# huj31415/nbody3d-webgpu

Hardware: AMD Instinct MI355X
Metric: pair-interactions/s (higher is better)
Workload: dtype f32; 1 GPU; N=262144 Plummer sphere, dt=1e-3, G=1, eps2=1e-4, i-sharded over 1 GPU(s); n=262144, kernel_variant=f32pk_symw_ipl16_j1_w2048_r32t128, parallelism=1gpu

## Files before the change

include/nbody3d_hip.h:

```cpp
#ifndef NBODY3D_HIP_H
#define NBODY3D_HIP_H

#include <stddef.h>
#include <stdint.h>

#ifdef __cplusplus
extern "C" {
#endif
#if defined(__GNUC__)
#pragma GCC visibility push(default)
#endif

#define NB_ABI_VERSION 2u
#define NB_ABI_MINOR 4u

typedef struct nb_sim nb_sim;

typedef enum nb_status {
    NB_OK = 0,
    NB_ERR_INVALID = 1,
    NB_ERR_NO_DEVICE = 2,
    NB_ERR_HIP = 3,
    NB_ERR_STATE = 4,
    NB_ERR_NOMEM = 5,
    NB_ERR_COMM = 6,
    NB_NOT_READY = 7
} nb_status;

typedef enum nb_precision { NB_F32 = 0, NB_F64 = 1 } nb_precision;

#define NB_FLAG_EXT_STREAM 1u
#define NB_FLAG_LDS_ONLY 4u
#define NB_FLAG_NO_FUSE 8u
#define NB_FLAG_POISON 16u

#define NB_FLAG_JPK_FENCED 32u

#define NB_FLAG_NO_SYM 64u

#define NB_FLAG_SYM_SHARD 128u

#define NB_FLAG_WHOLE_SWEEPS 256u

#define NB_FLAG_SINGLE_SWEEPS 512u

typedef enum nb_array { NB_BODIES = 0, NB_VEL = 1, NB_ACCEL = 2, NB_JERK = 3  } nb_array;

typedef enum nb_integrator { NB_INT_LEAPFROG = 0, NB_INT_HERMITE4 = 1 } nb_integrator;

typedef struct nb_config {
    uint32_t struct_size;
    uint32_t n;
    uint32_t precision;
    uint32_t tile;
    double eps2;
    int32_t device;
    uint32_t shard_begin;
    uint32_t shard_count;
    void *ext_stream;
    void *ext_bodies;
    uint32_t force_variant;
    uint32_t jsplit;
    uint32_t flags;
    uint32_t layer_budget_mib;
    uint32_t integrator;
    uint32_t reserved[3];
} nb_config;
// ... 55 lines not shown

int nb_enable_timing(nb_sim *s, int on);
int nb_kernel_times(nb_sim *s, double *force_ms, double *integrate_ms,
                    uint32_t *launches);
int nb_step_times(nb_sim *s, double *force_ms, double *integrate_ms, double *exchange_ms,
                  uint32_t *launches);
typedef struct nb_step_timing {
    uint32_t struct_size;
    uint32_t launches;
    double force_ms;
    double sym_reduce_ms;
    double reduce_scatter_ms;
    double integrate_ms;
    double allgather_ms;
    double span_ms;
    uint32_t reduce_scatters;
    uint32_t allgathers;
} nb_step_timing;
int nb_step_times2(nb_sim *s, nb_step_timing *out);
int nb_integrate_pass(nb_sim *s, uint32_t reps, double *avg_ms);
int nb_force_pass(nb_sim *s, uint32_t reps, double *avg_ms);

const char *nb_variant_name(nb_sim *s);

int nb_shape_info(nb_sim *s, uint32_t *jsplit, uint32_t *j_per_split, uint32_t *own_split0,
                  uint32_t *own_splits);



int nb_download_jerk(nb_sim *s, void *jerk);

int nb_upload_derivs(nb_sim *s, const void *accel, const void *jerk);

#define NB_BLOCK_FROZEN 1u
typedef struct nb_block_steps {
    uint32_t struct_size;
    uint32_t max_level;
    uint32_t min_level;
    uint32_t flags;
    double   eta;
} nb_block_steps;
int nb_set_block_steps(nb_sim *s, const nb_block_steps *cfg );

struct nb_block_stats {
    uint32_t struct_size, enabled;
    uint64_t outer_steps, block_steps, body_steps;
// ... 55 lines not shown
```

nbody3d-webgpu_amd/csrc/kernels/symmetric.hip.h:

```cpp
#pragma once

namespace nb {

template <typename T> struct SymRowT { T x, y, z; };
using SymRow = SymRowT<float>;

constexpr uint32_t kFlushSteps = 4096;

template <int NG>
__device__ __forceinline__ void flush_resident_sums(float (*hi)[64], const int lane, const bool flushed, nb_f2 (&ax)[NG], nb_f2 (&ay)[NG], nb_f2 (&az)[NG])
{
    if (flushed) {
#pragma unroll
        for (int c = 0; c < NG; ++c) {
            hi[6 * c + 0][lane] += ax[c].x; hi[6 * c + 1][lane] += ay[c].x; hi[6 * c + 2][lane] += az[c].x;
            hi[6 * c + 3][lane] += ax[c].y; hi[6 * c + 4][lane] += ay[c].y; hi[6 * c + 5][lane] += az[c].y;
        }
    } else {
#pragma unroll
        for (int c = 0; c < NG; ++c) {
            hi[6 * c + 0][lane] = ax[c].x; hi[6 * c + 1][lane] = ay[c].x; hi[6 * c + 2][lane] = az[c].x;
            hi[6 * c + 3][lane] = ax[c].y; hi[6 * c + 4][lane] = ay[c].y; hi[6 * c + 5][lane] = az[c].y;
        }
    }
#pragma unroll
    for (int c = 0; c < NG; ++c) { ax[c] = nb_f2{0, 0}; ay[c] = nb_f2{0, 0}; az[c] = nb_f2{0, 0}; }
}

__device__ __forceinline__ float wave_rot1(float v)
{
// ... 151 lines not shown
template <int TAIL>
__device__ __forceinline__ void symw_record_and_tail(const uint32_t* rec_at, nb_u4& rec, uint32_t (&tail)[TAIL])
{
    static_assert(TAIL == 1 || TAIL == 4, "f32: eps2; f64: G, eps2");
    constexpr int kTailOffset = 4 * 8 + 6 * 4;
    if constexpr (TAIL == 1) {
        asm volatile("s_load_dwordx4 %0, %2, 0x0\n\ts_load_dword %1, %3, %4\n\ts_waitcnt lgkmcnt(0)"
                     : "=&s"(rec), "=&s"(tail[0]) : "s"(rec_at), "s"(__builtin_amdgcn_kernarg_segment_ptr()), "n"(kTailOffset) : "memory");
    } else {
        nb_u4 t;
        asm volatile("s_load_dwordx4 %0, %2, 0x0\n\ts_load_dwordx4 %1, %3, %4\n\ts_waitcnt lgkmcnt(0)"
                     : "=&s"(rec), "=&s"(t) : "s"(rec_at), "s"(__builtin_amdgcn_kernarg_segment_ptr()), "n"(kTailOffset) : "memory");
        tail[0] = t.x; tail[1] = t.y; tail[2] = t.z; tail[3] = t.w;
    }
}

__device__ __forceinline__ SymWK symw_plan_words(uint32_t S, uint32_t cps, uint32_t W, uint32_t ups, uint32_t nsb, uint32_t zc, uint32_t r_layer0, uint32_t t_layer0)
{
    const uint32_t H = (nsb - 1u) >> 1, n_hi = (nsb & 1u) ? 0u : nsb >> 1;
    const uint32_t total_lo = (H + 1u) * cps + zc, total_hi = total_lo + (n_hi ? cps : 0u);
    return SymWK{(nsb + (zc ? 1u : 0u)) * S, nsb, W, total_hi, total_lo, n_hi, zc, ups, r_layer0, t_layer0};
}

template <int NG, int J, bool PAIR>
__device__ __forceinline__ void symw_sweeps(const uint32_t* __restrict__ gtab, const float4* __restrict__ bodies, SymRow* __restrict__ partial, SymRow* __restrict__ spill,
                                            SYMW_PLAN_PARAMS, uint32_t* __restrict__ queue, const uint32_t npieces, const uint32_t pieces_off)
{
    static_assert(!PAIR || J == 1, "paired sweeps: one traveler per lane and sweep");
    constexpr uint32_t S = 128u * NG;
    constexpr int GW = NG < 4 ? NG : 4;
    constexpr uint32_t CH = 64u * J;
    constexpr uint32_t CPS = S / CH;
    const SymWK pl = symw_plan_words(S, CPS, W_, ups_, nsb_, zc_, r_layer0_, t_layer0_);
    const int lane = threadIdx.x & 63, wi = threadIdx.x >> 6;
    const uint32_t w = __builtin_amdgcn_readfirstlane(blockIdx.x * 4u + wi);
    const bool active = w < pl.W;
    NB_STAMP(0);
    __shared__ float red[4][6 * NG][64];
    __shared__ uint32_t fin[4];
    const uint32_t ups = pl.ups, ush = (uint32_t)__builtin_ctz(ups), ustep = 64u >> ush,
                   tab1 = 2u * (pl.np / S);
    nb_u4 rec;
    uint32_t tail[1];
    symw_record_and_tail(gtab + tab1 + 4u * (active ? w : 0u), rec, tail);
    const float eps2 = __builtin_bit_cast(float, tail[0]);
    const nb_f2 e2 = nb_f2{eps2, eps2};
    const uint32_t first_lo = pl.n_hi * pl.total_hi, first_z = first_lo + (pl.nsb - pl.n_hi) * pl.total_lo;
    const uint32_t slot = rec.w;
    NB_STAMP_LIGHT(1);
    bool first_part = true;

    auto run = [&](uint32_t u, const uint32_t uend, const uint32_t piece_layer) -> uint32_t {
        uint32_t gfin = ~0u;
        while (u < uend) {
            const uint32_t p = u >> ush;
            uint32_t g, k, total;
            if (p < first_lo) { g = p / pl.total_hi; k = p - g * pl.total_hi; total = pl.total_hi; }
            else if (p < first_z) { const uint32_t r = p - first_lo; g = pl.n_hi + r / pl.total_lo; k = r - (g - pl.n_hi) * pl.total_lo; total = pl.total_lo; }
            else { g = pl.nsb; k = p - first_z; total = pl.zc; }
            const uint32_t ring = g < pl.nsb ? total - CPS - pl.zc : 0u;
            const uint32_t both_end = g < pl.nsb ? ring + pl.zc : 0u;
            uint32_t ug_end = (p - k + total) * ups;
// ... 25 lines not shown
                    since = 0;
                }
                since += pair ? 128u : s1 - s0;
                const bool sym = k < both_end, zsweep = k >= ring && sym;
                const uint32_t d = k / CPS;
                uint32_t tb = g + 1 + d;
                if (tb >= pl.nsb) tb -= pl.nsb;
                const uint32_t tstart = k < ring ? tb * S + (k % CPS) * CH : zsweep ? pl.nsb * S + (k - ring) * CH : g * S + (k - both_end) * CH;
                const uint32_t zrow = g * pl.zc + (k - ring);
                ++k;
                if constexpr (PAIR) {
                    if (pair) {
                        const bool zsweep1 = k >= ring;
                        const uint32_t d1 = k / CPS;
                        uint32_t tb1 = g + 1 + d1;
                        if (tb1 >= pl.nsb) tb1 -= pl.nsb;
                        const uint32_t tstart1 = zsweep1 ? pl.nsb * S + (k - ring) * CH : tb1 * S + (k % CPS) * CH;
                        const uint32_t zrow1 = g * pl.zc + (k - ring);
                        ++k;
                        const float4 t0 = ld4(bodies + tstart + lane), t1 = ld4(bodies + tstart1 + lane);
                        nb_f2 tx = nb_f2{t0.x, t1.x}, ty = nb_f2{t0.y, t1.y}, tz = nb_f2{t0.z, t1.z}, tm = nb_f2{t0.w, t1.w};
                        float bx0 = 0, bx1 = 0, by0 = 0, by1 = 0, bz0 = 0, bz1 = 0;
                        if (first_part) NB_STAMP(2);
                        for (uint32_t st = 0; st < 64u; ++st) {
                            nb_f2 sx = nb_f2{0, 0}, sy = nb_f2{0, 0}, sz = nb_f2{0, 0};
#pragma unroll
                            for (int c0g = 0; c0g < NG; c0g += GW) {
#pragma unroll
                                for (int f = 0; f < 2; ++f) {
                                    nb_f2 dx[GW], dy[GW], dz[GW], d2[GW], r[GW], si[GW], sj[GW];
#pragma unroll
                                    for (int c = 0; c < GW; ++c) dx[c] = symw_sub(f, tx, xi[c0g + c]);
#pragma unroll
                                    for (int c = 0; c < GW; ++c) dy[c] = symw_sub(f, ty, yi[c0g + c]);
#pragma unroll
                                    for (int c = 0; c < GW; ++c) dz[c] = symw_sub(f, tz, zi[c0g + c]);
#pragma unroll
                                    for (int c = 0; c < GW; ++c) d2[c] = __builtin_elementwise_fma(dx[c], dx[c], e2);
#pragma unroll
                                    for (int c = 0; c < GW; ++c) d2[c] = __builtin_elementwise_fma(dy[c], dy[c], d2[c]);
#pragma unroll
                                    for (int c = 0; c < GW; ++c) d2[c] = __builtin_elementwise_fma(dz[c], dz[c], d2[c]);
#pragma unroll
                                    for (int c = 0; c < GW; ++c) r[c] = d2[c] * d2[c];
#pragma unroll
                                    for (int c = 0; c < GW; ++c) r[c] = r[c] * d2[c];
// ... 180 lines not shown
            if (id >= npieces) break;
            const uint32_t pu = gtab[pieces_off + 2u * id], ll = gtab[pieces_off + 2u * id + 1u];
            (void)run(pu, pu + (ll >> 16), ll & 0xffffu);
        }
    }
    NB_STAMP(4);
}

#define SYMW_KERNEL_PARAMS const uint32_t* __restrict__ gtab, const float4* __restrict__ bodies, SymRow* __restrict__ partial, SymRow* __restrict__ spill, \
                           SYMW_PLAN_PARAMS, const float eps2_arg ,                       \
                           uint32_t* __restrict__ queue, const uint32_t npieces, const uint32_t pieces_off
#define SYMW_KERNEL_ARGS gtab, bodies, partial, spill, W_, ups_, nsb_, zc_, r_layer0_, t_layer0_, queue, npieces, pieces_off
template <int NG, int J>
__global__ __launch_bounds__(256) __attribute__((amdgpu_waves_per_eu(NG >= 4 ? 2 : 4, NG > 4 ? 2 : (NG < 4 ? 8 : 4))))
void nb_force_symw(SYMW_KERNEL_PARAMS)
{
    symw_sweeps<NG, J, false>(SYMW_KERNEL_ARGS);
}
template <int NG>
__global__ __launch_bounds__(256) __attribute__((amdgpu_waves_per_eu(2, NG > 4 ? 2 : 4)))
void nb_force_symw_pairs(SYMW_KERNEL_PARAMS)
{
    symw_sweeps<NG, 1, true>(SYMW_KERNEL_ARGS);
}

__device__ __forceinline__ double wave_rot1(double v)
{
    const long long b = __builtin_bit_cast(long long, v);
    const int lo = (int)(b & 0xffffffffll), hi = (int)(b >> 32);
    const unsigned rlo = (unsigned)__builtin_amdgcn_update_dpp(lo, lo, 0x13C, 0xF, 0xF, false);
    const unsigned rhi = (unsigned)__builtin_amdgcn_update_dpp(hi, hi, 0x13C, 0xF, 0xF, false);
    return __builtin_bit_cast(double, (long long)(((unsigned long long)rhi << 32) | rlo));
}

template <int IPL>
__global__ __launch_bounds__(256) __attribute__((amdgpu_waves_per_eu(2, 2)))
void nb_force_symw64(const uint32_t* __restrict__ gtab, const double4* __restrict__ bodies, SymRowT<double>* __restrict__ partial, SymRowT<double>* __restrict__ spill,
                     SYMW_PLAN_PARAMS, const double G_arg, const double eps2_arg ,
                     uint32_t* __restrict__ queue, const uint32_t npieces, const uint32_t pieces_off)
{
    constexpr uint32_t S = 64u * IPL, CH = 64u, CPS = S / CH;
    const SymWK pl = symw_plan_words(S, CPS, W_, ups_, nsb_, zc_, r_layer0_, t_layer0_);
    constexpr int GW = 4;
    const int lane = threadIdx.x & 63, wi = threadIdx.x >> 6;
    const uint32_t w = __builtin_amdgcn_readfirstlane(blockIdx.x * 4u + wi);
    const bool active = w < pl.W;
// ... 596 lines not shown
```

nbody3d-webgpu_amd/csrc/nb_engine.hip:

```cpp
#include "nb_internal.h"
#include "nb_kernels.hip.h"
#include "../../include/nbody3d_hip_plan.h"

#include <hip/hip_ext.h>

#include <algorithm>
#include <cmath>
#include <cstdio>
#include <cstdlib>
#include <cstring>
#include <new>
#include <type_traits>

namespace {
thread_local std::string g_create_error = "";
}

namespace nbi {
int fail(nb_sim* s, int code, const std::string& msg)
{
    if (s) s->err = msg; else g_create_error = msg;
    return code;
}
void set_create_error(const std::string& msg) { g_create_error = msg; }
// ... 70 lines not shown
    }
    if (ipl != 1) return nullptr;
    if (ls == 4) return (const void*)&nb::nb_force<T, 1, 4>;
    if (ls == 16) return (const void*)&nb::nb_force<T, 1, 16>;
    if (ls == 64) return (const void*)&nb::nb_force<T, 1, 64>;
    return nullptr;
}

const void* sgpr_kernel(int ipl, int ws)
{
    if (ipl == 4 && ws == 5) return (const void*)&nb::nb_force_pk_sgpr<2, 4, true>;
    if (ipl == 4) return ws == 4 ? (const void*)&nb::nb_force_pk_sgpr<2, 4> : (const void*)&nb::nb_force_pk_sgpr<2, 1>;
    if (ipl == 8 && ws == 5) return (const void*)&nb::nb_force_pk_sgpr<4, 4, true>;
    if (ipl == 8) return ws == 4 ? (const void*)&nb::nb_force_pk_sgpr<4, 4> : (const void*)&nb::nb_force_pk_sgpr<4, 1>;
    return nullptr;
}

const void* rank_kernel_of(bool f64, int ipl)
{
    if (f64) return ipl == 8 ? (const void*)&nb::nb_force_symw64_rank<8> : nullptr;
    return ipl == 16 ? (const void*)&nb::nb_force_symw_rank<8> : ipl == 8 ? (const void*)&nb::nb_force_symw_rank<4> : nullptr;
}

const void* kernel_of(bool f64, const Shape& sh, bool single_sweeps = false)
{
    switch (sh.kind) {
        case kScalar: return f64 ? scalar_kernel<double>(sh.ipl, sh.ls) : scalar_kernel<float>(sh.ipl, sh.ls);
        case kPkLds: return f64 || (sh.ipl & 1) ? nullptr : pk_force_kernel(sh.ipl / 2, sh.ls, sh.x);
        case kFused: return f64 || (sh.ipl & 1) ? nullptr : pk_fused_kernel(sh.ipl / 2, sh.ls, sh.x);
        case kPkSgpr: return f64 || sh.ls != 1 || !(sh.x == 1 || sh.x == 4 || sh.x == 5) ? nullptr : sgpr_kernel(sh.ipl, sh.x);
        case kDirect:
            if (f64 || sh.ipl != 2 || sh.ls != 64) return nullptr;
            return sh.x == 1 ? (const void*)&nb::nb_step_direct<16> : sh.x == 2 ? (const void*)&nb::nb_step_direct<32> : nullptr;
        case kSym:
            if (sh.ls != 1) return nullptr;
            if (f64) return sh.ipl == 8 && sh.x == 3 ? (const void*)&nb::nb_force_symw64<8> : nullptr;
            if (sh.x == 4) return sh.ipl == 8 ? (const void*)&nb::nb_force_sym<4, 4, 2> : nullptr;
            if (sh.ipl == 4) return sh.x == 3 ? (const void*)&nb::nb_force_symw<2, 1> : nullptr;
            if (sh.ipl == 8 && sh.x == 3) return single_sweeps ? (const void*)&nb::nb_force_symw<4, 1> : (const void*)&nb::nb_force_symw_pairs<4>;
            if (sh.ipl == 16 && sh.x == 3) return single_sweeps ? (const void*)&nb::nb_force_symw<8, 1> : (const void*)&nb::nb_force_symw_pairs<8>;
            if (sh.ipl == 8) return sh.x == 1 ? (const void*)&nb::nb_force_symw<4, 2> : nullptr;
            if (sh.ipl == 16) return sh.x == 1 ? (const void*)&nb::nb_force_symw<8, 2> : nullptr;
            return nullptr;
        case kJpk:
            if (f64 || sh.ipl != 1 || sh.ls != 1) return nullptr;
            return sh.x == 4 ? (const void*)&nb::nb_step_jpk<4> : sh.x == 8 ? (const void*)&nb::nb_step_jpk<8>
                   : sh.x == 6 ? (const void*)&nb::nb_step_jpk<16> : nullptr;
        default: return nullptr;
    }
}

void plan_handle(nb_sim* s, const nb_config& cfg, int n_cu, double clock_hz, double device_mem)
{
    PlanInput in;
    if (device_mem > 0) in.device_mem = device_mem;
    in.n = s->n; in.sb = s->sb; in.sc = s->sc; in.f64 = s->f64; in.cfg = cfg; in.n_cu = n_cu; in.clock_hz = clock_hz;
    if (!s->no_device)
        in.occupancy = [f64 = s->f64](const Shape& sh, int block) {
            int occ = 0;
            const void* fn = kernel_of(f64, sh);
            if (!fn || hipOccupancyMaxActiveBlocksPerMultiprocessor(&occ, fn, block, 0) != hipSuccess) { (void)hipGetLastError(); return 0; }
            return occ;
        };
// ... 82 lines not shown
            float e2 = (float)s->eps2;
            void* args[] = {&b, &p, &tab, &rp, &n, &e2, &w0, &w1, &sp, &k_lo, &k_hi, &d0};
            launch_kernel(rank_kernel_of(false, sh.ipl), dim3(ceil_div(w1 - w0, 4u)), dim3(256), args, s->stream, t0, t1);
        }
        return;
    }
    if (s->symw) {
        nb::SymWPlan pl;
        memcpy(&pl, s->sym_plan, sizeof pl);
        const void* b = jstream(s, s->cur);
        void* p = s->partial;
        const uint32_t* tab = s->sym_tab;
        void* sp = s->sym_spill;
        uint32_t* queue = s->sym_queue;
        uint32_t npieces = s->sym_pieces, pieces_off = 2u * (pl.np / ipb_of(sh)) + 4u * pl.W;
        if (npieces) (void)hipMemsetAsync(queue, 0, sizeof(uint32_t), s->stream);
        if (s->f64) {
            double G = s->G, e2 = s->eps2;
            void* args[] = {&tab, &b, &p, &sp, &pl.W, &pl.ups, &pl.nsb, &pl.zc, &pl.r_layer0, &pl.t_layer0, &G, &e2, &queue, &npieces, &pieces_off};
            launch_kernel(kernel_of(true, sh), dim3(ceil_div(pl.W, 4u)), dim3(256), args, s->stream, t0, t1);
        } else {
            float e2 = (float)s->eps2;
            void* args[] = {&tab, &b, &p, &sp, &pl.W, &pl.ups, &pl.nsb, &pl.zc, &pl.r_layer0, &pl.t_layer0, &e2, &queue, &npieces, &pieces_off};
            launch_kernel(kernel_of(false, sh, s->single_sweeps), dim3(ceil_div(pl.W, 4u)), dim3(256), args, s->stream, t0, t1);
        }
        return;
    }
    if (s->sym) {
        nb::SymPlan pl;
        memcpy(&pl, s->sym_plan, sizeof pl);
        const float4* b = (const float4*)jstream(s, s->cur);
        nb::SymRow* p = (nb::SymRow*)s->partial;
        float e2 = (float)s->eps2;
        uint32_t n = s->n;
        void* args[] = {&b, &p, &pl, &n, &e2};
        launch_kernel(kernel_of(false, sh), dim3(pl.nsb * pl.q), dim3(64 * sh.x), args, s->stream, t0, t1);
        return;
    }
    nb::SplitWindow win{0, 0xffffffffu, 0};
    uint32_t ny = s->jsplit;
    if (part == 1) { win.base = s->own_split0; ny = s->own_splits; }
    else if (part == 2) { win.hole_begin = s->own_split0; win.hole_count = s->own_splits; ny = s->jsplit - s->own_splits; }
    if (ny == 0) return;
    dim3 grid(ceil_div(s->sc, ipb_of(sh)), ny), block(nb::kBlock);
    const V4* b = (const V4*)jstream(s, s->cur);
    V4* p = (V4*)s->partial;
    T G = (T)s->G, e2 = (T)s->eps2;
// ... 540 lines not shown
        NB_HIPC(hipMemsetAsync(s->zero_row, 0, 64, s->stream));
        s->diag_chunk = nb::kTile * std::min(16u, std::max(1u, s->n / 16384u));
        s->diag_blocks = ceil_div(s->sc, nb::kDiagRows) * ceil_div(s->n, s->diag_chunk);
        NB_HIPC(hipMalloc((void**)&s->diag, sizeof(double) * 5 * s->diag_blocks));
        *out = s;
        return NB_OK;
    }
    plan_handle(s, cfg, n_cu, clock_hz, (double)prop.totalGlobalMem);
    if (s->sym && (!s->sym_rank || s->sym_local) && !cfg.force_variant) {
        size_t free_b = 0, total_b = 0;
        auto need = [&]() { return 3.0 * s->esz * (double)sym_layer_rows(s) * s->sym_layers + 12.0 * s->esz * s->sym_np; };
        if (hipMemGetInfo(&free_b, &total_b) == hipSuccess && need() > 0.9 * (double)free_b) {
            nb_config fit = cfg;
            fit.layer_budget_mib = (uint32_t)std::max(1.0, 0.6 * (double)free_b / 1048576.0);
            plan_handle(s, fit, n_cu, clock_hz, (double)prop.totalGlobalMem);
            if (s->sym && need() > 0.9 * (double)free_b) {
                cfg.flags |= NB_FLAG_NO_SYM;
                plan_handle(s, cfg, n_cu, clock_hz, (double)prop.totalGlobalMem);
            }
        }
    }
    if (!kernel_of(s->f64, shape_of(s))) return bail(NB_ERR_INVALID, "nb_create: no kernel for shape " + s->variant);
    s->single_sweeps = (cfg.flags & NB_FLAG_SINGLE_SWEEPS) != 0;

    const size_t row = 4 * s->esz;
    if (cfg.ext_bodies) { s->bodies[0] = cfg.ext_bodies; s->own_bodies = false; }
    else {
        const size_t rows = s->sym ? s->sym_np : s->n;
        NB_HIPC(hipMalloc(&s->bodies[0], row * rows));
        if (s->sym) NB_HIPC(hipMemset(s->bodies[0], 0, row * rows));
        s->own_bodies = true;
        if (s->fused) NB_HIPC(hipMalloc(&s->bodies[1], row * s->n));
    }
    NB_HIPC(hipMalloc(&s->vel, row * s->sc));
    NB_HIPC(hipMalloc(&s->acc, row * s->sc));
    auto alloc_partial = [&](size_t bytes) -> hipError_t {
        if (s->partial) return hipErrorInvalidValue;
        s->partial_bytes = bytes;
        return hipMalloc(&s->partial, bytes);
    };
    if (s->sym) {
        NB_HIPC(alloc_partial((size_t)3 * s->esz * sym_layer_rows(s) * s->sym_layers));
        if (s->sym_rank) NB_HIPC(hipMalloc(&s->sym_A, 4 * s->esz * s->sym_np));
        if (s->sym_spill_rows) {
            NB_HIPC(hipMalloc(&s->sym_spill, (size_t)3 * s->esz * s->sym_spill_rows));
            NB_HIPC(hipMemset(s->sym_spill, 0, (size_t)3 * s->esz * s->sym_spill_rows));
// ... 514 lines not shown
    auto once = [&]() -> int {
        if (s->hermite) { launch_fj(s, s->bodies[0], s->vel, s->hx, s->hv); return NB_OK; }
        if (s->sym_rank) return s->f64 ? nbi::sym_rank_phase_a_t<double>(s, nullptr, false) : nbi::sym_rank_phase_a_t<float>(s, nullptr, false);
        if (s->f64) launch_force<double>(s); else launch_force<float>(s);
        return NB_OK;
    };
    hipEvent_t e0, e1;
    NB_HIP(s, hipEventCreate(&e0));
    NB_HIP(s, hipEventCreate(&e1));
    if (int rc = once()) return rc;
    NB_HIP(s, hipEventRecord(e0, s->stream));
    for (uint32_t k = 0; k < reps; ++k) { if (int rc = once()) return rc; }
    NB_HIP(s, hipEventRecord(e1, s->stream));
    NB_HIP(s, hipEventSynchronize(e1));
    float ms = 0;
    NB_HIP(s, hipEventElapsedTime(&ms, e0, e1));
    (void)hipEventDestroy(e0); (void)hipEventDestroy(e1);
    NB_HIP(s, hipGetLastError());
    *avg_ms = ms / reps;
    return NB_OK;
}

const char* nb_variant_name(nb_sim* s) { return s ? s->variant.c_str() : ""; }

int nb_shape_info(nb_sim* s, uint32_t* jsplit, uint32_t* j_per_split, uint32_t* own_split0, uint32_t* own_splits)
{
    if (!s) return NB_ERR_INVALID;
    if (jsplit) *jsplit = s->jsplit;
    if (j_per_split) *j_per_split = s->j_per_split;
    if (own_split0) *own_split0 = s->own_split0;
    if (own_splits) *own_splits = s->own_splits;
    return NB_OK;
}

int nb_plan_query(const nb_config* cfg_in, int n_cu, double clock_hz, nb_plan_info* out, uint32_t* tab, uint32_t tab_cap)
{
    if (!cfg_in || !out) return fail(nullptr, NB_ERR_INVALID, "nb_plan_query: null argument");
    if (out->struct_size < sizeof(nb_plan_info)) return fail(nullptr, NB_ERR_INVALID, "nb_plan_query: set out->struct_size to sizeof(nb_plan_info)");
    nb_config cfg;
    uint32_t sb, sc;
    double eps2;
    if (const int rc = read_config(cfg_in, "nb_plan_query", &cfg, &sb, &sc, &eps2)) return rc;
    if (cfg.integrator != NB_INT_LEAPFROG) return fail(nullptr, NB_ERR_INVALID, "nb_plan_query: integrator must be NB_INT_LEAPFROG (a Hermite handle has no launch plan: nb_shape_info reports its j-chunks)");
    int count = 0;
    double device_mem = 0.0;
    if (hipGetDeviceCount(&count) != hipSuccess) { (void)hipGetLastError(); count = 0; }
// ... 405 lines not shown
```

nbody3d-webgpu_amd/csrc/nb_internal.h:

```cpp
#pragma once
#include "../../include/nbody3d_hip.h"
#include "nb_plan.h"

#include <hip/hip_runtime.h>

#include <cstdint>
#include <string>
#include <vector>

struct nb_events { hipEvent_t e[8]; bool two, xchg, rs, blk; };

struct nb_rccl;

struct nb_frame_slot {
    float* h_bodies = nullptr;
    float* h_speed = nullptr;
    float* d_bodies = nullptr;
    float* d_speed = nullptr;
    hipEvent_t packed = nullptr;
    hipEvent_t landed = nullptr;
    uint64_t step = 0;
    bool in_flight = false, valid = false;
};

// ... 31 lines not shown
    bool direct = false;
    bool jpk = false;
    void* pairs[2] = {nullptr, nullptr};
    bool pairs_ok = false;
    double pairs_G = 0.0;
    void* jpartial = nullptr;
    uint32_t* tickets = nullptr;
    uint32_t junits = 0;
    bool poison = false;
    bool jpk_fenced = false;
    int acc_parity = 0;
    bool swap_acc = false;
    uint32_t jsplit = 1, j_per_split = 0;
    bool sym = false;
    uint32_t sym_np = 0, sym_layers = 0;
    uint32_t sym_plan[16] = {0};
    bool symw = false;
    uint32_t* sym_tab = nullptr;
    std::vector<uint32_t> sym_tab_host;
    void* sym_spill = nullptr;
    uint32_t sym_spill_rows = 0;
    uint32_t sym_pieces = 0;
    bool single_sweeps = false;
    uint32_t* sym_queue = nullptr;
    bool sym_rank = false;
    uint32_t sym_g0 = 0, sym_g1 = 0;
    uint32_t sym_rank_plan[16] = {0};
    std::vector<nbp::LaunchPlan::SymPass> sym_passes;
    uint32_t sym_pass = 0;
    bool sym_local = false;
    void* sym_A = nullptr;
    std::string variant, err;
    nb_exchange_fn xfn = nullptr;
    nb_exchange_wait_fn xwait = nullptr;
    void* xuser = nullptr;
    bool gather_pending = false;
    uint32_t own_split0 = 0, own_splits = 0;
    nb_rccl* rccl = nullptr;
    bool timing = false;
    struct graph_slot {
        hipGraph_t graph = nullptr;
        hipGraphExec_t exec = nullptr;
        double dt = 0.0, G = 0.0;
        int parity = 0;
    } graphs[2];
    bool graphs_ok = true;
// ... 50 lines not shown
```

nbody3d-webgpu_amd/nbody3d_amd/capi.py:

```python
import ctypes as C
import os

import numpy as np

_PKG = os.path.dirname(os.path.abspath(__file__))
_LIB_PATH = os.environ.get("NB_ENGINE_LIB") or os.path.normpath(os.path.join(_PKG, "..", "csrc", "libnbody3d_hip.so"))

NB_F32, NB_F64 = 0, 1
NB_FLAG_EXT_STREAM = 1
NB_FLAG_LDS_ONLY = 4
NB_FLAG_NO_FUSE = 8
NB_FLAG_POISON = 16
NB_FLAG_JPK_FENCED = 32
NB_FLAG_NO_SYM = 64
NB_FLAG_SYM_SHARD = 128
NB_FLAG_WHOLE_SWEEPS = 256
NB_FLAG_SINGLE_SWEEPS = 512
NB_RCCL_ID_BYTES = 128
NB_RCCL_OVERLAP = 1
NB_MULTI_PEER, NB_MULTI_RCCL, NB_MULTI_PEER_OVERLAP = 0, 1, 2
NB_NOT_READY = 7
NB_FIELD_AT_BODIES, NB_FIELD_F64, NB_FIELD_DEVICE = 1, 2, 4
NB_NBR_AT_BODIES, NB_NBR_DEVICE = 1, 4
NB_NBR_NONE = 0xffffffff
NB_INT_LEAPFROG, NB_INT_HERMITE4 = 0, 1
INTEGRATORS = {"leapfrog": NB_INT_LEAPFROG, "hermite4": NB_INT_HERMITE4}
STATUS = {0: "NB_OK", 1: "NB_ERR_INVALID", 2: "NB_ERR_NO_DEVICE", 3: "NB_ERR_HIP",
          4: "NB_ERR_STATE", 5: "NB_ERR_NOMEM", 6: "NB_ERR_COMM", 7: "NB_NOT_READY"}
ABI_VERSION = 2
ABI_MINOR = 3


class NBodyError(RuntimeError):
    def __init__(self, code, msg):
        super().__init__("%s: %s" % (STATUS.get(code, code), msg))
        self.code = code


class nb_config(C.Structure):
    _fields_ = [
# ... 39 lines not shown
    _fields_ = [("struct_size", C.c_uint32), ("max_level", C.c_uint32), ("min_level", C.c_uint32), ("flags", C.c_uint32),
                ("eta", C.c_double)]


class nb_block_stats(C.Structure):
    _fields_ = [("struct_size", C.c_uint32), ("enabled", C.c_uint32), ("outer_steps", C.c_uint64), ("block_steps", C.c_uint64),
                ("body_steps", C.c_uint64), ("clamped", C.c_uint64), ("finest_level", C.c_uint32), ("reserved", C.c_uint32)]


EXCHANGE_FN = C.CFUNCTYPE(C.c_int, C.c_void_p, C.c_void_p, C.c_size_t, C.c_uint32, C.c_uint32, C.c_uint32, C.c_void_p)
EXCHANGE_WAIT_FN = C.CFUNCTYPE(C.c_int, C.c_void_p, C.c_void_p)

SYMBOLS = ["nb_abi_version", "nb_device_count", "nb_create", "nb_destroy", "nb_upload", "nb_set_params", "nb_step",
           "nb_download", "nb_sync", "nb_last_error", "nb_device_ptr", "nb_set_exchange",
           "nb_set_exchange_overlapped", "nb_enable_timing",
           "nb_kernel_times", "nb_variant_name", "nb_diagnostics",
           "nb_multi_create", "nb_multi_destroy", "nb_multi_upload", "nb_multi_set_params", "nb_multi_step",
           "nb_multi_download", "nb_multi_sync", "nb_multi_last_error", "nb_multi_variant_name",
           "nb_multi_diagnostics", "nb_multi_set_collective", "nb_multi_collective_info",
           "nb_rccl_unique_id", "nb_rccl_attach", "nb_rccl_detach", "nb_rccl_info",
           "nb_step_times", "nb_step_times2", "nb_integrate_pass", "nb_force_pass", "nb_frame_request", "nb_frame_acquire", "nb_shape_info", "nb_plan_query",
           "nb_abi_minor", "nb_field_eval", "nb_multi_field_eval", "nb_download_jerk", "nb_upload_derivs",
           "nb_set_block_steps", "nb_block_stats", "nb_download_levels", "nb_upload_levels",
           "nb_neighbors", "nb_multi_neighbors", "nb_neighbors_shape"]

_lib = None


def library_path():
    return _LIB_PATH


def load_library():
    global _lib
    if _lib is not None:
        return _lib
    if not os.path.exists(_LIB_PATH):
        raise NBodyError(3, "HIP engine not built: %s is missing (run __graft_entry__.build() or "
                            "make -C nbody3d-webgpu_amd/csrc)" % _LIB_PATH)
    L = C.CDLL(_LIB_PATH)
    vp = C.c_void_p
    L.nb_abi_version.restype = C.c_uint32
    L.nb_abi_minor.restype = C.c_uint32
    L.nb_device_count.restype = C.c_int
    L.nb_create.argtypes = [C.POINTER(nb_config), C.POINTER(vp)]
    L.nb_destroy.argtypes = [vp]
    L.nb_destroy.restype = None
# ... 32 lines not shown
    L.nb_rccl_detach.argtypes = [vp]
    L.nb_rccl_info.argtypes = [vp, C.POINTER(C.c_int), C.POINTER(C.c_int), C.POINTER(C.c_int)]
    L.nb_step_times.argtypes = [vp, C.POINTER(C.c_double), C.POINTER(C.c_double), C.POINTER(C.c_double),
                                C.POINTER(C.c_uint32)]
    L.nb_step_times2.argtypes = [vp, C.POINTER(nb_step_timing)]
    L.nb_integrate_pass.argtypes = [vp, C.c_uint32, C.POINTER(C.c_double)]
    L.nb_force_pass.argtypes = [vp, C.c_uint32, C.POINTER(C.c_double)]
    L.nb_shape_info.argtypes = [vp] + [C.POINTER(C.c_uint32)] * 4
    L.nb_plan_query.argtypes = [C.POINTER(nb_config), C.c_int, C.c_double, C.POINTER(nb_plan_info), C.POINTER(C.c_uint32), C.c_uint32]
    L.nb_frame_request.argtypes = [vp]
    L.nb_frame_acquire.argtypes = [vp, C.c_int, C.POINTER(C.POINTER(C.c_float)), C.POINTER(C.POINTER(C.c_float)),
                                   C.POINTER(C.c_uint64)]
    if L.nb_abi_minor() >= 4:
        L.nb_field_eval.argtypes = [vp, C.POINTER(nb_field_request)]
        L.nb_multi_field_eval.argtypes = [vp, C.POINTER(nb_field_request)]
    if hasattr(L, "nb_download_jerk"):
        L.nb_download_jerk.argtypes = [vp, vp]
        L.nb_upload_derivs.argtypes = [vp, vp, vp]
    if hasattr(L, "nb_set_block_steps"):
        L.nb_set_block_steps.argtypes = [vp, C.POINTER(nb_block_steps)]
        L.nb_block_stats.argtypes = [vp, C.POINTER(nb_block_stats), C.c_int]
        L.nb_download_levels.argtypes = [vp, vp]
        L.nb_upload_levels.argtypes = [vp, vp]
    if hasattr(L, "nb_neighbors"):
        L.nb_neighbors.argtypes = [vp, C.POINTER(nb_neighbor_request)]
        L.nb_multi_neighbors.argtypes = [vp, C.POINTER(nb_neighbor_request)]
        L.nb_neighbors_shape.argtypes = [vp, C.c_uint32] + [C.POINTER(C.c_uint32)] * 3
    _lib = L
    return L


def abi_version():
    return load_library().nb_abi_version()


def abi_minor():
    return load_library().nb_abi_minor()


def device_count():
    return load_library().nb_device_count()


def rccl_unique_id():
    L = load_library()
    buf = C.create_string_buffer(NB_RCCL_ID_BYTES)
# ... 411 lines not shown

    def rccl_info(self):
        a, b, c = C.c_int(), C.c_int(), C.c_int()
        self._check(self._L.nb_rccl_info(self._h, C.byref(a), C.byref(b), C.byref(c)))
        return a.value, b.value, c.value

    def request_frame(self):
        self._check(self._L.nb_frame_request(self._h))

    def frame(self, wait=True):
        pb, ps, st = C.POINTER(C.c_float)(), C.POINTER(C.c_float)(), C.c_uint64()
        rc = self._L.nb_frame_acquire(self._h, 1 if wait else 0, C.byref(pb), C.byref(ps), C.byref(st))
        if rc == NB_NOT_READY:
            return None
        self._check(rc)
        b = np.ctypeslib.as_array(pb, shape=(self.n, 4))
        sp = np.ctypeslib.as_array(ps, shape=(self.n,))
        return b, sp, st.value

    @property
    def variant(self):
        return self._L.nb_variant_name(self._h).decode()

    def shape_info(self):
        v = [C.c_uint32() for _ in range(4)]
        self._check(self._L.nb_shape_info(self._h, *[C.byref(x) for x in v]))
        return dict(zip(("jsplit", "j_per_split", "own_split0", "own_splits"), (x.value for x in v)))

    def diagnostics(self):
        out = (C.c_double * 5)()
        self._check(self._L.nb_diagnostics(self._h, out))
        return out[0], out[1], np.array(out[2:5])

    def field(self, points=None, *, bodies=None, accel=True, phi=True, f64=False):
        req, pts, a, f = _field_request(self.n, self.dtype, points, bodies, accel, phi, f64)
        self._check(self._L.nb_field_eval(self._h, C.byref(req)))
        return a, f

    def field_device(self, points_ptr, m, accel_ptr, phi_ptr, *, bodies=None, f64=False):
        if self._L.nb_abi_minor() < 4:
            raise NBodyError(1, "field_device(): the loaded library is ABI %d.%d; nb_field_eval needs 2.4" % (abi_version(), abi_minor()))
        req = nb_field_request()
        req.struct_size = C.sizeof(nb_field_request)
        req.flags = NB_FIELD_DEVICE | (NB_FIELD_F64 if f64 else 0)
        if bodies is not None:
            req.flags |= NB_FIELD_AT_BODIES
# ... 178 lines not shown
```

Measured before the change: 6835 billion pair-interactions/s.

## Rotate paired-sweep travelers through LDS instead of DPP lane rotations

Adds a new default kernel for the ipl=16 paired symmetric sweeps. It writes each wave's traveler bodies into a doubled LDS ring and reads the rotated rows by sliding an address, instead of moving the traveler coordinates between lanes with DPP rotations at every step. The loop is unrolled by two, with hand-placed LDS loads, sched barriers and waitcnts so the next traveler load overlaps the current pair computation. The launch pins occupancy at two waves per EU. It adds LDS usage and leaves the old DPP path behind a new flag.

```diff
diff --git a/include/nbody3d_hip.h b/include/nbody3d_hip.h
--- a/include/nbody3d_hip.h
+++ b/include/nbody3d_hip.h
@@ -43,6 +43,8 @@
 #define NB_FLAG_WHOLE_SWEEPS 256u
 
 #define NB_FLAG_SINGLE_SWEEPS 512u
+
+#define NB_FLAG_DPP_TRAVELERS 1024u
 
 typedef enum nb_array { NB_BODIES = 0, NB_VEL = 1, NB_ACCEL = 2, NB_JERK = 3  } nb_array;
 
@@ -144,6 +146,7 @@
 int nb_force_pass(nb_sim *s, uint32_t reps, double *avg_ms);
 
 const char *nb_variant_name(nb_sim *s);
+const char *nb_force_form(const nb_sim *s);
 
 int nb_shape_info(nb_sim *s, uint32_t *jsplit, uint32_t *j_per_split, uint32_t *own_split0,
                   uint32_t *own_splits);
diff --git a/nbody3d-webgpu_amd/csrc/kernels/symmetric.hip.h b/nbody3d-webgpu_amd/csrc/kernels/symmetric.hip.h
--- a/nbody3d-webgpu_amd/csrc/kernels/symmetric.hip.h
+++ b/nbody3d-webgpu_amd/csrc/kernels/symmetric.hip.h
@@ -6,6 +6,7 @@
 using SymRow = SymRowT<float>;
 
 constexpr uint32_t kFlushSteps = 4096;
+constexpr uint32_t kTravRows = 127;
 
 template <int NG>
 __device__ __forceinline__ void flush_resident_sums(float (*hi)[64], const int lane, const bool flushed, nb_f2 (&ax)[NG], nb_f2 (&ay)[NG], nb_f2 (&az)[NG])
@@ -203,11 +204,12 @@
     return SymWK{(nsb + (zc ? 1u : 0u)) * S, nsb, W, total_hi, total_lo, n_hi, zc, ups, r_layer0, t_layer0};
 }
 
-template <int NG, int J, bool PAIR>
+template <int NG, int J, bool PAIR, bool LT = false>
 __device__ __forceinline__ void symw_sweeps(const uint32_t* __restrict__ gtab, const float4* __restrict__ bodies, SymRow* __restrict__ partial, SymRow* __restrict__ spill,
                                             SYMW_PLAN_PARAMS, uint32_t* __restrict__ queue, const uint32_t npieces, const uint32_t pieces_off)
 {
     static_assert(!PAIR || J == 1, "paired sweeps: one traveler per lane and sweep");
+    static_assert(!LT || PAIR, "travelers from LDS: the paired sweeps only");
     constexpr uint32_t S = 128u * NG;
     constexpr int GW = NG < 4 ? NG : 4;
     constexpr uint32_t CH = 64u * J;
@@ -219,6 +221,11 @@
     NB_STAMP(0);
     __shared__ float red[4][6 * NG][64];
     __shared__ uint32_t fin[4];
+    [[maybe_unused]] uint32_t trav_at = 0;
+    if constexpr (LT) {
+        __shared__ nb_v4f trav[4][2][kTravRows];
+        trav_at = (uint32_t)(uintptr_t)(__attribute__((address_space(3))) nb_v4f*)&trav[wi][0][0];
+    }
     const uint32_t ups = pl.ups, ush = (uint32_t)__builtin_ctz(ups), ustep = 64u >> ush,
                    tab1 = 2u * (pl.np / S);
     nb_u4 rec;
@@ -290,6 +297,86 @@
                         nb_f2 tx = nb_f2{t0.x, t1.x}, ty = nb_f2{t0.y, t1.y}, tz = nb_f2{t0.z, t1.z}, tm = nb_f2{t0.w, t1.w};
                         float bx0 = 0, bx1 = 0, by0 = 0, by1 = 0, bz0 = 0, bz1 = 0;
                         if (first_part) NB_STAMP(2);
+                        if constexpr (LT) {
+                            auto pair_step = [&](const nb_f2 tx, const nb_f2 ty, const nb_f2 tz, const nb_f2 tm, nb_f2& sx, nb_f2& sy, nb_f2& sz) {
+#pragma unroll
+                                for (int c0g = 0; c0g < NG; c0g += GW) {
+#pragma unroll
+                                    for (int f = 0; f < 2; ++f) {
+                                        nb_f2 dx[GW], dy[GW], dz[GW], d2[GW], r[GW], si[GW], sj[GW];
+#pragma unroll
+                                        for (int c = 0; c < GW; ++c) dx[c] = symw_sub(f, tx, xi[c0g + c]);
+#pragma unroll
+                                        for (int c = 0; c < GW; ++c) dy[c] = symw_sub(f, ty, yi[c0g + c]);
+#pragma unroll
+                                        for (int c = 0; c < GW; ++c) dz[c] = symw_sub(f, tz, zi[c0g + c]);
+#pragma unroll
+                                        for (int c = 0; c < GW; ++c) d2[c] = __builtin_elementwise_fma(dx[c], dx[c], e2);
+#pragma unroll
+                                        for (int c = 0; c < GW; ++c) d2[c] = __builtin_elementwise_fma(dy[c], dy[c], d2[c]);
+#pragma unroll
+                                        for (int c = 0; c < GW; ++c) d2[c] = __builtin_elementwise_fma(dz[c], dz[c], d2[c]);
+#pragma unroll
+                                        for (int c = 0; c < GW; ++c) r[c] = d2[c] * d2[c];
+#pragma unroll
+                                        for (int c = 0; c < GW; ++c) r[c] = r[c] * d2[c];
+#pragma unroll
+                                        for (int c = 0; c < GW; ++c) r[c] = nb_f2{nb_rsq(r[c].x), nb_rsq(r[c].y)};
+#pragma unroll
+                                        for (int c = 0; c < GW; ++c) si[c] = symw_mul(f, tm, r[c]);
+#pragma unroll
+                                        for (int c = 0; c < GW; ++c) sj[c] = mi[c0g + c] * r[c];
+#pragma unroll
+                                        for (int c = 0; c < GW; ++c) ax[c0g + c] = __builtin_elementwise_fma(si[c], dx[c], ax[c0g + c]);
+#pragma unroll
+                                        for (int c = 0; c < GW; ++c) ay[c0g + c] = __builtin_elementwise_fma(si[c], dy[c], ay[c0g + c]);
+#pragma unroll
+                                        for (int c = 0; c < GW; ++c) az[c0g + c] = __builtin_elementwise_fma(si[c], dz[c], az[c0g + c]);
+#pragma unroll
+                                        for (int c = 0; c < GW; ++c) sx = symw_fnma(f, sj[c], dx[c], sx);
+#pragma unroll
+                                        for (int c = 0; c < GW; ++c) sy = symw_fnma(f, sj[c], dy[c], sy);
+#pragma unroll
+                                        for (int c = 0; c < GW; ++c) sz = symw_fnma(f, sj[c], dz[c], sz);
+                                    }
+                                }
+                            };
+                            auto sums_on = [&](const nb_f2 sx, const nb_f2 sy, const nb_f2 sz) {
+                                wave_rot1_add(bx0, sx.x); wave_rot1_add(bx1, sx.y); wave_rot1_add(by0, sy.x); wave_rot1_add(by1, sy.y);
+                                wave_rot1_add(bz0, sz.x); wave_rot1_add(bz1, sz.y);
+                            };
+                            using lds_f4 = __attribute__((address_space(3))) const nb_v4f;
+                            {
+                                using lds_w4 = __attribute__((address_space(3))) nb_v4f;
+                                lds_w4* ta = (lds_w4*)(uintptr_t)trav_at;
+                                const nb_v4f ra = nb_v4f{t0.x, t1.x, t0.y, t1.y}, rb = nb_v4f{t0.z, t1.z, t0.w, t1.w};
+                                ta[lane] = ra; ta[kTravRows + lane] = rb;
+                                if (lane < 63) { ta[64 + lane] = ra; ta[kTravRows + 64 + lane] = rb; }
+                            }
+                            uint32_t row = trav_at + 16u * (63u + (uint32_t)lane);
+                            for (uint32_t st = 0; st < 32u; ++st) {
+                                lds_f4* r1 = (lds_f4*)(uintptr_t)row;
+                                const nb_v4f a1 = r1[0], b1 = r1[kTravRows];
+                                __builtin_amdgcn_sched_barrier(0);
+                                nb_f2 sx = nb_f2{0, 0}, sy = nb_f2{0, 0}, sz = nb_f2{0, 0};
+                                pair_step(tx, ty, tz, tm, sx, sy, sz);
+                                sums_on(sx, sy, sz);
+                                __builtin_amdgcn_sched_barrier(0);
+                                __builtin_amdgcn_s_waitcnt(0xc07f);
+                                asm volatile("v_subrev_u32_e32 %0, 32, %0" : "+v"(row));
+                                lds_f4* r2 = (lds_f4*)(uintptr_t)row;
+                                const nb_v4f a2 = r2[1], b2 = r2[kTravRows + 1];
+                                __builtin_amdgcn_sched_barrier(0);
+                                sx = nb_f2{0, 0}; sy = nb_f2{0, 0}; sz = nb_f2{0, 0};
+                                pair_step(nb_f2{a1.x, a1.y}, nb_f2{a1.z, a1.w}, nb_f2{b1.x, b1.y}, nb_f2{b1.z, b1.w}, sx, sy, sz);
+                                sums_on(sx, sy, sz);
+                                __builtin_amdgcn_sched_barrier(0);
+                                __builtin_amdgcn_s_waitcnt(0xc07f);
+                                tx = nb_f2{a2.x, a2.y}; ty = nb_f2{a2.z, a2.w}; tz = nb_f2{b2.x, b2.y}; tm = nb_f2{b2.z, b2.w};
+                                __builtin_amdgcn_sched_barrier(0);
+                            }
+                        }
+                        if constexpr (!LT)
                         for (uint32_t st = 0; st < 64u; ++st) {
                             nb_f2 sx = nb_f2{0, 0}, sy = nb_f2{0, 0}, sz = nb_f2{0, 0};
 #pragma unroll
@@ -516,6 +603,13 @@
 void nb_force_symw_pairs(SYMW_KERNEL_PARAMS)
 {
     symw_sweeps<NG, 1, true>(SYMW_KERNEL_ARGS);
+}
+template <int NG>
+__global__ __launch_bounds__(256) __attribute__((amdgpu_waves_per_eu(2, 2)))
+void nb_force_symw_lt(SYMW_KERNEL_PARAMS)
+{
+    static_assert(NG == 8, "two waves per SIMD");
+    symw_sweeps<NG, 1, true, true>(SYMW_KERNEL_ARGS);
 }
 
 __device__ __forceinline__ double wave_rot1(double v)
diff --git a/nbody3d-webgpu_amd/csrc/nb_engine.hip b/nbody3d-webgpu_amd/csrc/nb_engine.hip
--- a/nbody3d-webgpu_amd/csrc/nb_engine.hip
+++ b/nbody3d-webgpu_amd/csrc/nb_engine.hip
@@ -116,7 +116,7 @@
     return ipl == 16 ? (const void*)&nb::nb_force_symw_rank<8> : ipl == 8 ? (const void*)&nb::nb_force_symw_rank<4> : nullptr;
 }
 
-const void* kernel_of(bool f64, const Shape& sh, bool single_sweeps = false)
+const void* kernel_of(bool f64, const Shape& sh, bool single_sweeps = false, bool dpp_travelers = false)
 {
     switch (sh.kind) {
         case kScalar: return f64 ? scalar_kernel<double>(sh.ipl, sh.ls) : scalar_kernel<float>(sh.ipl, sh.ls);
@@ -132,7 +132,7 @@
             if (sh.x == 4) return sh.ipl == 8 ? (const void*)&nb::nb_force_sym<4, 4, 2> : nullptr;
             if (sh.ipl == 4) return sh.x == 3 ? (const void*)&nb::nb_force_symw<2, 1> : nullptr;
             if (sh.ipl == 8 && sh.x == 3) return single_sweeps ? (const void*)&nb::nb_force_symw<4, 1> : (const void*)&nb::nb_force_symw_pairs<4>;
-            if (sh.ipl == 16 && sh.x == 3) return single_sweeps ? (const void*)&nb::nb_force_symw<8, 1> : (const void*)&nb::nb_force_symw_pairs<8>;
+            if (sh.ipl == 16 && sh.x == 3) return single_sweeps ? (const void*)&nb::nb_force_symw<8, 1> : dpp_travelers ? (const void*)&nb::nb_force_symw_pairs<8> : (const void*)&nb::nb_force_symw_lt<8>;
             if (sh.ipl == 8) return sh.x == 1 ? (const void*)&nb::nb_force_symw<4, 2> : nullptr;
             if (sh.ipl == 16) return sh.x == 1 ? (const void*)&nb::nb_force_symw<8, 2> : nullptr;
             return nullptr;
@@ -261,7 +261,7 @@
         } else {
             float e2 = (float)s->eps2;
             void* args[] = {&tab, &b, &p, &sp, &pl.W, &pl.ups, &pl.nsb, &pl.zc, &pl.r_layer0, &pl.t_layer0, &e2, &queue, &npieces, &pieces_off};
-            launch_kernel(kernel_of(false, sh, s->single_sweeps), dim3(ceil_div(pl.W, 4u)), dim3(256), args, s->stream, t0, t1);
+            launch_kernel(kernel_of(false, sh, s->single_sweeps, s->dpp_travelers), dim3(ceil_div(pl.W, 4u)), dim3(256), args, s->stream, t0, t1);
         }
         return;
     }
@@ -848,6 +848,7 @@
     }
     if (!kernel_of(s->f64, shape_of(s))) return bail(NB_ERR_INVALID, "nb_create: no kernel for shape " + s->variant);
     s->single_sweeps = (cfg.flags & NB_FLAG_SINGLE_SWEEPS) != 0;
+    s->dpp_travelers = (cfg.flags & NB_FLAG_DPP_TRAVELERS) != 0;
 
     const size_t row = 4 * s->esz;
     if (cfg.ext_bodies) { s->bodies[0] = cfg.ext_bodies; s->own_bodies = false; }
@@ -1408,6 +1409,11 @@
 }
 
 const char* nb_variant_name(nb_sim* s) { return s ? s->variant.c_str() : ""; }
+const char* nb_force_form(const nb_sim* s)
+{
+    if (!s || !s->symw || s->f64 || s->ws != 3 || (s->ipl != 8 && s->ipl != 16)) return "";
+    return s->single_sweeps ? "dpp-single" : (s->ipl == 16 && !s->dpp_travelers) ? "lds-pairs" : "dpp-pairs";
+}
 
 int nb_shape_info(nb_sim* s, uint32_t* jsplit, uint32_t* j_per_split, uint32_t* own_split0, uint32_t* own_splits)
 {
diff --git a/nbody3d-webgpu_amd/csrc/nb_internal.h b/nbody3d-webgpu_amd/csrc/nb_internal.h
--- a/nbody3d-webgpu_amd/csrc/nb_internal.h
+++ b/nbody3d-webgpu_amd/csrc/nb_internal.h
@@ -77,6 +77,7 @@
     uint32_t sym_spill_rows = 0;
     uint32_t sym_pieces = 0;
     bool single_sweeps = false;
+    bool dpp_travelers = false;
     uint32_t* sym_queue = nullptr;
     bool sym_rank = false;
     uint32_t sym_g0 = 0, sym_g1 = 0;
diff --git a/nbody3d-webgpu_amd/nbody3d_amd/capi.py b/nbody3d-webgpu_amd/nbody3d_amd/capi.py
--- a/nbody3d-webgpu_amd/nbody3d_amd/capi.py
+++ b/nbody3d-webgpu_amd/nbody3d_amd/capi.py
@@ -16,6 +16,7 @@
 NB_FLAG_SYM_SHARD = 128
 NB_FLAG_WHOLE_SWEEPS = 256
 NB_FLAG_SINGLE_SWEEPS = 512
+NB_FLAG_DPP_TRAVELERS = 1024
 NB_RCCL_ID_BYTES = 128
 NB_RCCL_OVERLAP = 1
 NB_MULTI_PEER, NB_MULTI_RCCL, NB_MULTI_PEER_OVERLAP = 0, 1, 2
@@ -101,7 +102,7 @@
            "nb_step_times", "nb_step_times2", "nb_integrate_pass", "nb_force_pass", "nb_frame_request", "nb_frame_acquire", "nb_shape_info", "nb_plan_query",
            "nb_abi_minor", "nb_field_eval", "nb_multi_field_eval", "nb_download_jerk", "nb_upload_derivs",
            "nb_set_block_steps", "nb_block_stats", "nb_download_levels", "nb_upload_levels",
-           "nb_neighbors", "nb_multi_neighbors", "nb_neighbors_shape"]
+           "nb_neighbors", "nb_multi_neighbors", "nb_neighbors_shape", "nb_force_form"]
 
 _lib = None
 
@@ -180,6 +181,9 @@
         L.nb_block_stats.argtypes = [vp, C.POINTER(nb_block_stats), C.c_int]
         L.nb_download_levels.argtypes = [vp, vp]
         L.nb_upload_levels.argtypes = [vp, vp]
+    if hasattr(L, "nb_force_form"):
+        L.nb_force_form.argtypes = [vp]
+        L.nb_force_form.restype = C.c_char_p
     if hasattr(L, "nb_neighbors"):
         L.nb_neighbors.argtypes = [vp, C.POINTER(nb_neighbor_request)]
         L.nb_multi_neighbors.argtypes = [vp, C.POINTER(nb_neighbor_request)]
@@ -637,6 +641,12 @@
     def variant(self):
         return self._L.nb_variant_name(self._h).decode()
 
+    @property
+    def force_form(self):
+        if not hasattr(self._L, "nb_force_form"):
+            raise NBodyError(1, "force_form: the loaded library has no nb_force_form")
+        return self._L.nb_force_form(self._h).decode()
+
     def shape_info(self):
         v = [C.c_uint32() for _ in range(4)]
         self._check(self._L.nb_shape_info(self._h, *[C.byref(x) for x in v]))
```

New measurement: 6884 billion pair-interactions/s (median of 6 runs). About the same (+0.7%).
